# linjieli222/HERO

Measured on AMD Instinct MI355X. Metric: videos/sec training step, HERO-base TVR-shaped batch, higher is better.
Workload: dtype bf16; 1 GPU; configs[1]: HERO-base TVR finetune micro-step (train-tvr-8gpu.json shapes: 32 videos x 60 frames, 15 subs x (4 frames + 20 tokens), 15-token query; vfeat 4352; fwd + VSM loss + bwd, all-reduce/clip/AdamW every 2nd micro-step); global_batch=32, parallelism=dp1, grad_accum=2, launch=hipGraph replay, input=one batch resident in HBM

## Files before the change

hero_amd/_lib.py:

```python
import ctypes as C
import os

import torch

_HERE = os.path.dirname(os.path.abspath(__file__))
LIB_PATH = os.environ.get("HERO_HIP_LIB") or os.path.join(_HERE, "libhero_hip.so")

ABI_VERSION = 3
F32, BF16 = 0, 1
LAYOUT_K, LAYOUT_O = 0, 1
ACT_NONE, ACT_GELU, ACT_RELU, ACT_GELU_BWD, ACT_RELU_BWD, ACT_GELU_DG, ACT_MUL_AUX = 0, 1, 2, 3, 4, 5, 6

EXPORTS = [
    "hero_last_error", "hero_abi_version", "hero_abi_struct_count", "hero_abi_struct_bytes", "hero_gemm", "hero_gemm_splits", "hero_fold_slabs", "hero_wgrad_group", "hero_wgrad_batch_plan", "hero_wgrad_batch", "hero_prof_enable", "hero_prof_read", "hero_probe_mfma", "hero_probe_hbm", "hero_gemm_force_config", "hero_layernorm_fwd",
    "hero_layernorm_bwd_workspace_bytes", "hero_layernorm_bwd", "hero_colsum_workspace_bytes",
    "hero_colsum", "hero_colsum_multi", "hero_colsum_multi_workspace_bytes", "hero_layernorm_bwd_blocks", "hero_attention_fwd", "hero_attention_bwd", "hero_attention_max_len", "hero_attention_max_packed_len", "hero_attention_stats_ok", "hero_attention_force_ppw",
    "hero_gather_rows", "hero_inverse_first", "hero_csr_gather_sum", "hero_scatter_add_rows", "hero_segment_sort_workspace_bytes", "hero_scatter_add_sorted_workspace_bytes", "hero_segment_sort", "hero_scatter_add_sorted", "hero_cast", "hero_transpose_cast", "hero_copy_multi",
    "hero_relu_bwd", "hero_gelu_bwd", "hero_add", "hero_sumsq", "hero_adamw", "hero_adamw_multi", "hero_adamw_multi_chunk",
    "hero_query_pool_fwd", "hero_query_pool_bwd", "hero_rownorm_fwd", "hero_rownorm_bwd", "hero_score_max_fwd",
    "hero_score_max_bwd", "hero_rank_loss", "hero_sums_scaled", "hero_st_ed_fwd", "hero_st_ed_bwd", "hero_st_ed_bwd_workspace_bytes",
    "hero_cross_entropy_fwd", "hero_cross_entropy_bwd", "hero_qa_pool_fwd", "hero_qa_pool_bwd",
    "hero_topk_rows", "hero_st_ed_probs", "hero_moment_topk", "hero_moment_nms", "hero_first_hit",
    "hero_collate_subs", "hero_collate_clip_mask", "hero_collate_frame_map", "hero_collate_gather_feats", "hero_derive_multi",
    "hero_comm_available", "hero_comm_unique_id", "hero_comm_init", "hero_comm_destroy", "hero_comm_rank", "hero_comm_world",
    "hero_comm_allreduce_buckets", "hero_comm_broadcast", "hero_comm_allgather", "hero_comm_allgather_var",
]


class Dropout(C.Structure):
    _fields_ = [("seed_ptr", C.c_void_p), ("site", C.c_uint64),
                ("threshold16", C.c_uint32), ("scale", C.c_float)]


class GemmEpilogue(C.Structure):
    _fields_ = [("bias", C.c_void_p), ("residual", C.c_void_p), ("aux", C.c_void_p),
                ("act", C.c_int), ("out_f32", C.c_int), ("beta", C.c_float),
                ("split_k", C.c_int), ("dropout", Dropout), ("colsum", C.c_void_p), ("colsum_partial", C.c_int), ("pad_", C.c_int), ("split_stride", C.c_longlong)]


class CrossEntropy(C.Structure):
    _fields_ = [("logits", C.c_void_p), ("labels", C.c_void_p), ("loss", C.c_void_p), ("lse", C.c_void_p),
                ("dloss", C.c_void_p), ("dlogits", C.c_void_p), ("rows", C.c_int), ("cols", C.c_int),
                ("ld", C.c_int), ("dtype", C.c_int), ("inv_temp", C.c_float), ("ignore_index", C.c_int64)]


class Derive(C.Structure):
    _fields_ = [("src", C.c_void_p), ("dst", C.c_void_p), ("n", C.c_int64), ("mode", C.c_int), ("p0", C.c_int),
                ("p1", C.c_int), ("p2", C.c_int)]

# ... 113 lines not shown
    return {st.__name__: C.sizeof(st) for st in ABI_STRUCTS}


_lib = None


def lib():
    global _lib
    if _lib is None:
        if not os.path.exists(LIB_PATH):
            raise RuntimeError(
                "hero_amd: %s is missing. Build it with `python -m hero_amd.build` "
                "(needs hipcc; cross-compiles for gfx950 without a GPU). There is no fallback "
                "path." % LIB_PATH)
        L = C.CDLL(LIB_PATH)
        L.hero_last_error.restype = C.c_char_p
        have = L.hero_abi_version()
        if have != ABI_VERSION:
            raise RuntimeError("hero_amd: %s reports ABI version %d, this binding was written against %d (struct layouts "
                               "differ: rebuild with `python -m hero_amd.build --force`)" % (LIB_PATH, have, ABI_VERSION))
        L.hero_abi_struct_bytes.argtypes = [C.c_int]
        if L.hero_abi_struct_count() != len(ABI_STRUCTS):
            raise RuntimeError("hero_amd: %s declares %d ABI structs, this binding mirrors %d" % (LIB_PATH, L.hero_abi_struct_count(), len(ABI_STRUCTS)))
        bad = [(st.__name__, C.sizeof(st), L.hero_abi_struct_bytes(i)) for i, st in enumerate(ABI_STRUCTS)
               if C.sizeof(st) != L.hero_abi_struct_bytes(i)]
        if bad:
            raise RuntimeError("hero_amd: struct layouts differ from %s (name, binding bytes, library bytes): %s" % (LIB_PATH, bad))
        L.hero_layernorm_bwd_workspace_bytes.restype = C.c_size_t
        L.hero_colsum_workspace_bytes.restype = C.c_size_t
        L.hero_colsum_multi_workspace_bytes.restype = C.c_size_t
        L.hero_colsum_multi_workspace_bytes.argtypes = [C.POINTER(Colsum), C.c_int]
        L.hero_colsum_multi.argtypes = [C.POINTER(Colsum), C.c_int, C.c_void_p, C.c_void_p]
        L.hero_layernorm_bwd_blocks.argtypes = [C.c_int]
        L.hero_gemm.argtypes = [C.c_void_p, C.c_void_p, C.c_void_p] + [C.c_int] * 9 + [
            C.POINTER(GemmEpilogue), C.c_void_p]
        L.hero_gemm_splits.argtypes = [C.c_int, C.c_int, C.c_int]
        L.hero_fold_slabs.argtypes = [C.c_void_p, C.c_int, C.c_size_t, C.c_void_p, C.c_size_t, C.c_int, C.c_void_p]
        L.hero_wgrad_group.argtypes = [C.POINTER(WgradProblem), C.c_int, C.c_int, C.c_int, C.c_void_p]
        L.hero_wgrad_batch_plan.argtypes = [C.POINTER(WgradProblem), C.c_int, C.c_int, C.c_void_p, C.c_int]
        L.hero_wgrad_batch.argtypes = [C.POINTER(WgradProblem), C.c_int, C.c_int, C.c_int, C.c_void_p, C.c_int, C.c_void_p]
        L.hero_prof_enable.argtypes = [C.c_int]
        L.hero_prof_read.argtypes = [C.c_int, C.POINTER(C.c_double), C.POINTER(C.c_double),
                                     C.POINTER(C.c_longlong)]
        L.hero_probe_mfma.argtypes = [C.c_void_p, C.c_size_t, C.POINTER(C.c_double), C.POINTER(C.c_double), C.c_void_p]
        L.hero_probe_hbm.argtypes = [C.c_void_p, C.c_void_p, C.c_size_t, C.POINTER(C.c_double), C.POINTER(C.c_double), C.c_void_p]
        L.hero_layernorm_fwd.argtypes = [C.POINTER(LnFwd), C.c_void_p]
        L.hero_layernorm_bwd.argtypes = [C.POINTER(LnBwd), C.c_void_p]
        L.hero_layernorm_bwd_workspace_bytes.argtypes = [C.c_int, C.c_int]
        L.hero_colsum_workspace_bytes.argtypes = [C.c_int, C.c_int]
        L.hero_colsum.argtypes = [C.c_void_p, C.c_void_p, C.c_int, C.c_int, C.c_int, C.c_int,
                                  C.c_float, C.c_void_p, C.c_void_p]
        L.hero_attention_fwd.argtypes = [C.POINTER(Attn), C.c_void_p]
        L.hero_attention_bwd.argtypes = [C.POINTER(Attn), C.c_void_p]
        L.hero_attention_stats_ok.argtypes = [C.c_int, C.c_int]
        L.hero_attention_force_ppw.argtypes = [C.c_int]
        L.hero_attention_max_len.argtypes = [C.c_int, C.c_int]
        L.hero_attention_max_packed_len.argtypes = [C.c_int]
        L.hero_gather_rows.argtypes = [C.c_void_p, C.c_void_p, C.c_void_p, C.c_void_p,
                                       C.c_int, C.c_int, C.c_int, C.c_void_p]
        L.hero_inverse_first.argtypes = [C.c_void_p, C.c_int, C.c_void_p, C.c_int, C.c_int, C.c_void_p]
        L.hero_csr_gather_sum.argtypes = [C.c_void_p, C.c_void_p, C.c_void_p, C.c_void_p,
                                          C.c_int, C.c_int, C.c_int, C.c_void_p]
        L.hero_scatter_add_rows.argtypes = [C.c_void_p, C.c_void_p, C.c_void_p, C.c_void_p,
                                            C.c_int, C.c_int, C.c_int, C.c_int, C.c_int, C.c_void_p]
        L.hero_segment_sort_workspace_bytes.argtypes = [C.c_int]
        L.hero_segment_sort_workspace_bytes.restype = C.c_size_t
# ... 88 lines not shown
```

hero_amd/csrc/layernorm.hip:

```cpp
#include "common.h"

namespace hero {

__device__ __forceinline__ void add4(float4& s, const float4& v) { s.x += v.x; s.y += v.y; s.z += v.z; s.w += v.w; }
__device__ __forceinline__ void ln_mask4(float4& v, const DropCtx& drop, int row, int cols, int c) {
  const float4 m = drop.mask4(((uint64_t)row * (uint64_t)cols + (uint64_t)c) >> 2);
  v.x *= m.x; v.y *= m.y; v.z *= m.z; v.w *= m.w;
}

template <int VPL, int GRP>
__device__ __forceinline__ void ln_fwd_gamma_beta(const HeroLnFwd& a, const int (&cc)[VPL], int i0, float4 (&g)[GRP], float4 (&b)[GRP]) {
#pragma unroll
  for (int u = 0; u < GRP; ++u)
    if (i0 + u < VPL) {
      g[u] = *reinterpret_cast<const float4*>(a.gamma + cc[i0 + u]);
      b[u] = *reinterpret_cast<const float4*>(a.beta + cc[i0 + u]);
    }
}

template <typename TX, typename TY, int VPL, bool FULL>
__device__ __forceinline__ void ln_fwd_row(const HeroLnFwd& a, int row, int lane) {
  const int cols = FULL ? VPL * 256 : a.cols;
  int cc[VPL];
  float okf[VPL];
// ... 60 lines not shown
        const int i = i0 + u;
        o[u].x = (v[i].x - mean) * rstd * g[u].x + b[u].x;
        o[u].y = (v[i].y - mean) * rstd * g[u].y + b[u].y;
        o[u].z = (v[i].z - mean) * rstd * g[u].z + b[u].z;
        o[u].w = (v[i].w - mean) * rstd * g[u].w + b[u].w;
      }
    if (drop.on()) {
#pragma unroll
      for (int u = 0; u < GRP; ++u)
        if (i0 + u < VPL) ln_mask4(o[u], drop, row, cols, cc[i0 + u]);
    }
    if (pre) {
#pragma unroll
      for (int u = 0; u < GRP; ++u)
        if (i0 + u < VPL && (FULL || okf[i0 + u] != 0.f)) V4<TY>::st(pre + cc[i0 + u], v[i0 + u]);
    }
#pragma unroll
    for (int u = 0; u < GRP; ++u)
      if (i0 + u < VPL && (FULL || okf[i0 + u] != 0.f)) V4<TY>::st(y + cc[i0 + u], o[u]);
  }
}

template <typename TX, typename TY, int VPL>
__global__ __launch_bounds__(256) void ln_fwd_kernel(HeroLnFwd a) {
  const int lane = threadIdx.x & 63, row = blockIdx.x * 4 + (threadIdx.x >> 6);
  if (row < a.rows) ln_fwd_row<TX, TY, VPL, false>(a, row, lane);
}
template <typename TX, typename TY, int VPL>
__global__ __launch_bounds__(256) void ln_fwd_full_kernel(HeroLnFwd a) {
  const int lane = threadIdx.x & 63, row = blockIdx.x * 4 + (threadIdx.x >> 6);
  if (row < a.rows) ln_fwd_row<TX, TY, VPL, true>(a, row, lane);
}

template <typename TX, typename T, int VPL, bool FULL, bool ACC>
__device__ __forceinline__ void ln_bwd_row(const HeroLnBwd& a, int row, int lane, const DropCtx dout, const DropCtx din,
                                           const float4* gm, float4* ag, float4* ab, float4* ai) {
  const int cols = FULL ? VPL * 256 : a.cols;
  const float inv = 1.f / (float)cols;
  const TX* x = static_cast<const TX*>(a.x) + (size_t)row * cols;
  const T* dy = static_cast<const T*>(a.dy) + (size_t)row * cols;
  float4 xv[VPL], d[VPL];
  if constexpr (FULL) {
#pragma unroll
    for (int i = 0; i < VPL; ++i) {
      xv[i] = V4<TX>::ld(x + (lane + 64 * i) * 4);
      d[i] = V4<T>::ld(dy + (lane + 64 * i) * 4);
    }
  }
  const float mean = a.mean[row], rstd = a.rstd[row];
  if constexpr (FULL) {
    if (dout.on()) {
#pragma unroll
      for (int i = 0; i < VPL; ++i) ln_mask4(d[i], dout, row, cols, (lane + 64 * i) * 4);
    }
  }
  float4 xh[VPL], g[VPL];
  float s1 = 0.f, s2 = 0.f;
#pragma unroll
  for (int i = 0; i < VPL; ++i) {
    const int c = (lane + 64 * i) * 4;
    xh[i] = make_float4(0.f, 0.f, 0.f, 0.f);
    g[i] = xh[i];
    if (FULL || c < cols) {
      if constexpr (!FULL) {
        xv[i] = V4<TX>::ld(x + c);
        d[i] = V4<T>::ld(dy + c);
        if (dout.on()) ln_mask4(d[i], dout, row, cols, c);
      }
      const float4 gv = FULL ? gm[i] : *reinterpret_cast<const float4*>(a.gamma + c);
      xh[i] = make_float4((xv[i].x - mean) * rstd, (xv[i].y - mean) * rstd, (xv[i].z - mean) * rstd, (xv[i].w - mean) * rstd);
      g[i] = make_float4(d[i].x * gv.x, d[i].y * gv.y, d[i].z * gv.z, d[i].w * gv.w);
      if constexpr (ACC) {
        ag[i].x += d[i].x * xh[i].x; ag[i].y += d[i].y * xh[i].y; ag[i].z += d[i].z * xh[i].z; ag[i].w += d[i].w * xh[i].w;
        add4(ab[i], d[i]);
      }
      s1 += (g[i].x + g[i].y) + (g[i].z + g[i].w);
      s2 += (g[i].x * xh[i].x + g[i].y * xh[i].y) + (g[i].z * xh[i].z + g[i].w * xh[i].w);
    }
  }
  s1 = wave_sum(s1) * inv;
  s2 = wave_sum(s2) * inv;
  T* dx = a.dx ? static_cast<T*>(a.dx) + (size_t)row * cols : nullptr;
  T* dxd = a.dx_dropped ? static_cast<T*>(a.dx_dropped) + (size_t)row * cols : nullptr;
  constexpr int GRP = FULL ? VPL : 1;
#pragma unroll
  for (int i0 = 0; i0 < VPL; i0 += GRP) {
    if (!FULL && (lane + 64 * i0) * 4 >= cols) continue;
    float4 o[GRP];
#pragma unroll
    for (int u = 0; u < GRP; ++u) {
      const int i = i0 + u;
      o[u].x = rstd * (g[i].x - s1 - xh[i].x * s2);
      o[u].y = rstd * (g[i].y - s1 - xh[i].y * s2);
      o[u].z = rstd * (g[i].z - s1 - xh[i].z * s2);
      o[u].w = rstd * (g[i].w - s1 - xh[i].w * s2);
    }
    if (dx) {
#pragma unroll
      for (int u = 0; u < GRP; ++u) V4<T>::st(dx + (lane + 64 * (i0 + u)) * 4, o[u]);
    }
    if (din.on()) {
#pragma unroll
      for (int u = 0; u < GRP; ++u) ln_mask4(o[u], din, row, cols, (lane + 64 * (i0 + u)) * 4);
    }
    if (dxd) {
#pragma unroll
      for (int u = 0; u < GRP; ++u) V4<T>::st(dxd + (lane + 64 * (i0 + u)) * 4, o[u]);
    }
    if constexpr (ACC) {
#pragma unroll
      for (int u = 0; u < GRP; ++u) add4(ai[i0 + u], o[u]);
    }
  }
}

template <typename TX, typename T, int VPL>
__global__ __launch_bounds__(256) void ln_bwd_dx_kernel(HeroLnBwd a) {
  const int lane = threadIdx.x & 63, row = blockIdx.x * 4 + (threadIdx.x >> 6);
  if (row >= a.rows) return;
  DropCtx dout(a.dropout_out), din(a.dropout_in);
  ln_bwd_row<TX, T, VPL, false, false>(a, row, lane, dout, din, nullptr, nullptr, nullptr, nullptr);
}

template <typename TX, typename T, int VPL, bool FULL>
__device__ __forceinline__ void ln_bwd_fused(const HeroLnBwd& a, float* partial) {
  extern __shared__ __attribute__((aligned(16))) float red[];
  const int lane = threadIdx.x & 63, wave = threadIdx.x >> 6;
  const int cols = FULL ? VPL * 256 : a.cols;
  DropCtx dout(a.dropout_out), din(a.dropout_in);
  float4 ag[VPL], ab[VPL], ai[VPL], gm[VPL];
#pragma unroll
  for (int i = 0; i < VPL; ++i) {
    ag[i] = ab[i] = ai[i] = make_float4(0.f, 0.f, 0.f, 0.f);
    if constexpr (FULL) gm[i] = *reinterpret_cast<const float4*>(a.gamma + (lane + 64 * i) * 4);
  }
  for (int row = blockIdx.x * 4 + wave; row < a.rows; row += gridDim.x * 4)
    ln_bwd_row<TX, T, VPL, FULL, true>(a, row, lane, dout, din, gm, ag, ab, ai);
#pragma unroll
  for (int i = 0; i < VPL; ++i) {
    const int c = (lane + 64 * i) * 4;
    if (FULL || c < cols) {
      *reinterpret_cast<float4*>(red + ((size_t)(wave * 3 + 0)) * cols + c) = ag[i];
      *reinterpret_cast<float4*>(red + ((size_t)(wave * 3 + 1)) * cols + c) = ab[i];
      *reinterpret_cast<float4*>(red + ((size_t)(wave * 3 + 2)) * cols + c) = ai[i];
    }
  }
  __syncthreads();
  const int n4 = 3 * (cols >> 2);
  for (int q = threadIdx.x; q < n4; q += 256) {
    const int k = q / (cols >> 2), c = (q - k * (cols >> 2)) * 4;
    float4 v = *reinterpret_cast<const float4*>(red + (size_t)k * cols + c);
#pragma unroll
    for (int w = 1; w < 4; ++w) add4(v, *reinterpret_cast<const float4*>(red + ((size_t)(w * 3 + k)) * cols + c));
    *reinterpret_cast<float4*>(partial + ((size_t)blockIdx.x * 3 + k) * cols + c) = v;
  }
}

template <typename TX, typename T, int VPL>
__global__ __launch_bounds__(256) void ln_bwd_fused_kernel(HeroLnBwd a, float* partial) {
  ln_bwd_fused<TX, T, VPL, false>(a, partial);
}
template <typename TX, typename T, int VPL>
__global__ __launch_bounds__(256) __attribute__((amdgpu_waves_per_eu(4, 8))) void ln_bwd_fused_full_kernel(HeroLnBwd a, float* partial) {
  ln_bwd_fused<TX, T, VPL, true>(a, partial);
}

__global__ __launch_bounds__(256) void colred_final3_kernel(const float* partial, float* o0, float* o1, float* o2, int cols,
                                                            int nblocks, float beta) {
  const int k = blockIdx.y;
  float* out = k == 0 ? o0 : (k == 1 ? o1 : o2);
  if (!out) return;
  __shared__ float4 red[16][16];
  const int cg = threadIdx.x & 15, kl = threadIdx.x >> 4;
  const int c = (blockIdx.x * 16 + cg) * 4;
  float4 s = make_float4(0.f, 0.f, 0.f, 0.f);
  if (c < cols) {
    int b = kl;
    for (; b + 48 < nblocks; b += 64) {
      float4 v[4];
#pragma unroll
      for (int u = 0; u < 4; ++u) v[u] = *reinterpret_cast<const float4*>(partial + ((size_t)(b + 16 * u) * 3 + k) * cols + c);
#pragma unroll
      for (int u = 0; u < 4; ++u) add4(s, v[u]);
    }
    for (; b < nblocks; b += 16) add4(s, *reinterpret_cast<const float4*>(partial + ((size_t)b * 3 + k) * cols + c));
  }
  red[kl][cg] = s;
  __syncthreads();
  if (kl == 0 && c < cols) {
    float4 o = make_float4(0.f, 0.f, 0.f, 0.f);
    if (beta != 0.f) {
      o = *reinterpret_cast<const float4*>(out + c);
      o.x *= beta; o.y *= beta; o.z *= beta; o.w *= beta;
    }
#pragma unroll
    for (int j = 1; j < 16; ++j) add4(s, red[j][cg]);
    add4(o, s);
// ... 138 lines not shown
}

template <typename F>
static int ln_dtypes(const char* who, const char* second, int xd, int d, F f) {
  if (xd == HERO_F32 && d == HERO_F32) return f(float(), float());
  if (xd == HERO_F32 && d == HERO_BF16) return f(float(), bf16_t());
  if (xd == HERO_BF16 && d == HERO_BF16) return f(bf16_t(), bf16_t());
  set_error("%s: unsupported dtypes x=%d %s=%d", who, xd, second, d);
  return HERO_ERR_UNSUPPORTED;
}

#define HERO_VPL_SWITCH4(cols, CALL)                                       \
  do {                                                                     \
    const int need4 = ((cols) + 255) / 256;                                \
    if (need4 <= 1) { CALL(1); }                                           \
    else if (need4 <= 2) { CALL(2); }                                      \
    else if (need4 <= 3) { CALL(3); }                                      \
    else { CALL(4); }                                                      \
  } while (0)
#define HERO_VPL_SWITCH(cols, CALL)                                        \
  do {                                                                     \
    const int need = ((cols) + 255) / 256;                                 \
    if (need <= 4) HERO_VPL_SWITCH4(cols, CALL);                           \
    else if (need <= 6) { CALL(6); }                                       \
    else if (need <= 8) { CALL(8); }                                       \
    else if (need <= 12) { CALL(12); }                                     \
    else if (need <= 17) { CALL(17); }                                     \
    else if (need <= 24) { CALL(24); }                                     \
    else { set_error("layernorm: cols %d too wide (max 6144)", (cols)); return HERO_ERR_UNSUPPORTED; } \
  } while (0)

}

#define LN_BWD_MAX_BLOCKS 1024
using namespace hero;

extern "C" int hero_layernorm_fwd(const HeroLnFwd* a, hero_stream_t stream) {
  HERO_REQUIRE(a && a->y && a->gamma && a->beta, "hero_layernorm_fwd: null pointer");
  HERO_REQUIRE(a->x || a->tab[0] || a->tab[1] || a->tab[2], "hero_layernorm_fwd: no input");
  HERO_REQUIRE(a->cols > 0 && a->cols % 4 == 0, "hero_layernorm_fwd: cols (%d) must be a positive multiple of 4", a->cols);
  if (a->rows <= 0) return HERO_OK;
  hipStream_t s = static_cast<hipStream_t>(stream);
  const dim3 grid((a->rows + 3) / 4), block(256);
  const int xd = a->x ? a->x_dtype : a->y_dtype, yd = a->y_dtype;
  int rc = HERO_OK;
#define LAUNCH(KERNEL, V)                                                                         \
  rc = ln_dtypes("hero_layernorm_fwd", "y", xd, yd, [&](auto tx, auto ty) {                       \
    hipLaunchKernelGGL((KERNEL<decltype(tx), decltype(ty), V>), grid, block, 0, s, *a);           \
    return HERO_OK;                                                                               \
  })
  if (a->x && !a->tab[0] && !a->tab[1] && !a->tab[2] && a->cols % 256 == 0 && a->cols <= 1024) {
#define CALL(V) LAUNCH(ln_fwd_full_kernel, V)
    HERO_VPL_SWITCH4(a->cols, CALL);
#undef CALL
    return rc ? rc : check_launch("hero_layernorm_fwd(full)");
  }
#define CALL(V) LAUNCH(ln_fwd_kernel, V)
  HERO_VPL_SWITCH(a->cols, CALL);
#undef CALL
#undef LAUNCH
  return rc ? rc : check_launch("hero_layernorm_fwd");
}

extern "C" size_t hero_layernorm_bwd_workspace_bytes(int rows, int cols) {
  (void)rows;
  return (size_t)LN_BWD_MAX_BLOCKS * (size_t)cols * 3 * sizeof(float);
}
extern "C" size_t hero_colsum_workspace_bytes(int rows, int cols) {
  (void)rows;
  return (size_t)256 * (size_t)cols * sizeof(float);
}

extern "C" int hero_layernorm_bwd(const HeroLnBwd* a, hero_stream_t stream) {
  HERO_REQUIRE(a && a->x && a->dy && a->gamma && a->mean && a->rstd, "hero_layernorm_bwd: null pointer");
  HERO_REQUIRE(a->cols > 0 && a->cols % 4 == 0, "hero_layernorm_bwd: cols (%d) must be a positive multiple of 4", a->cols);
  if (a->rows <= 0) return HERO_OK;
  hipStream_t s = static_cast<hipStream_t>(stream);
  const int xd = a->x_dtype, d = a->dtype;
  const bool want_params = a->dgamma || a->dbeta || a->dbias_in;
  if (want_params) HERO_REQUIRE(a->workspace, "hero_layernorm_bwd: workspace required for parameter gradients");
  int rc = HERO_OK;
#define LAUNCH(KERNEL, V, LDS, ...)                                                                         \
  rc = ln_dtypes("hero_layernorm_bwd", "dy", xd, d, [&](auto tx, auto t) {                                  \
    hipLaunchKernelGGL((KERNEL<decltype(tx), decltype(t), V>), grid, block, LDS, s, __VA_ARGS__);          \
    return HERO_OK;                                                                                         \
  })
  if (want_params && (a->dx || a->dx_dropped || a->dbias_in) && a->cols <= 1024) {
    int nblk = (a->rows + 3) / 4;
    if (nblk > LN_BWD_MAX_BLOCKS) nblk = LN_BWD_MAX_BLOCKS;
    float* partial = static_cast<float*>(a->workspace);
    const size_t lds = (size_t)4 * 3 * a->cols * sizeof(float);
    const dim3 grid(nblk), block(256);
    if (a->cols % 256 == 0) {
#define CALL(V) LAUNCH(ln_bwd_fused_full_kernel, V, lds, *a, partial)
      HERO_VPL_SWITCH4(a->cols, CALL);
#undef CALL
    } else {
#define CALL(V) LAUNCH(ln_bwd_fused_kernel, V, lds, *a, partial)
      HERO_VPL_SWITCH4(a->cols, CALL);
#undef CALL
    }
    if (rc) return rc;
    rc = check_launch("hero_layernorm_bwd(fused)");
    if (rc || a->defer_fold) return rc;
    hipLaunchKernelGGL(colred_final3_kernel, dim3((a->cols + 63) / 64, 3), dim3(256), 0, s, partial, a->dgamma, a->dbeta,
                       a->dbias_in, a->cols, nblk, a->grad_beta);
    return check_launch("hero_layernorm_bwd(final3)");
  }
  HERO_REQUIRE(!a->dbias_in, "hero_layernorm_bwd: dbias_in needs cols <= 1024");
  HERO_REQUIRE(!a->defer_fold, "hero_layernorm_bwd: defer_fold needs the fused path (cols <= 1024, dx or dbias_in wanted)");
  if (a->dx || a->dx_dropped) {
    const dim3 grid((a->rows + 3) / 4), block(256);
#define CALL(V) LAUNCH(ln_bwd_dx_kernel, V, 0, *a)
    HERO_VPL_SWITCH(a->cols, CALL);
#undef CALL
    if (rc) return rc;
    rc = check_launch("hero_layernorm_bwd(dx)");
    if (rc) return rc;
  }
#undef LAUNCH
  if (a->dgamma || a->dbeta)
    return ln_dtypes("hero_layernorm_bwd", "dy", xd, d, [&](auto tx, auto t) {
      return run_colred<decltype(tx), decltype(t)>(a->x, a->dy, a->mean, a->rstd, a->dgamma, a->dbeta, a->rows, a->cols, a->cols,
                                                   a->grad_beta, a->dropout_out, a->workspace, s);
    });
  return HERO_OK;
}

extern "C" int hero_layernorm_bwd_blocks(int rows) {
  int nblk = (rows + 3) / 4;
  return nblk > LN_BWD_MAX_BLOCKS ? LN_BWD_MAX_BLOCKS : nblk;
}

struct ColsumMulti {
  HeroColsum p[HERO_COLSUM_MULTI_MAX];
  int blk0[HERO_COLSUM_MULTI_MAX + 1];
  int woff[HERO_COLSUM_MULTI_MAX];
  int rpc[HERO_COLSUM_MULTI_MAX];
  int n;
};

__device__ __forceinline__ int colsum_find(const ColsumMulti& a, int b) {
  int lo = 0, hi = a.n - 1;
  while (lo < hi) {
    const int mid = (lo + hi + 1) >> 1;
    if (a.blk0[mid] <= b) lo = mid; else hi = mid - 1;
  }
  return lo;
}

__global__ __launch_bounds__(256) void colsum_multi_part_kernel(ColsumMulti a, float* ws) {
  __shared__ float4 red[4][64];
  const int pi = colsum_find(a, blockIdx.x);
  const HeroColsum P = a.p[pi];
  const int ncb = (P.cols + 255) / 256;
  const int local = blockIdx.x - a.blk0[pi], cb = local % ncb, chunk = local / ncb;
  const int tx = threadIdx.x & 63, ty = threadIdx.x >> 6;
  const int c = (cb * 64 + tx) * 4;
  const int r0 = chunk * a.rpc[pi], r1 = min(P.rows, r0 + a.rpc[pi]);
  float4 s = make_float4(0.f, 0.f, 0.f, 0.f), unused = s;
  const float* const none = nullptr;
  if (c < P.cols) {
    if (P.dtype == HERO_BF16) colsum_chunk(static_cast<const bf16_t*>(P.src), P.ld, c, r0, r1, ty, s, none, none, none, 0, nullptr, unused);
    else colsum_chunk(static_cast<const float*>(P.src), P.ld, c, r0, r1, ty, s, none, none, none, 0, nullptr, unused);
// ... 98 lines not shown
```

hero_amd/functional.py:

```python
import ctypes as C
import math
import os
import weakref

import numpy as np
import torch

from . import _lib as L

_COMPUTE_DTYPE = torch.bfloat16


def set_compute_dtype(dtype):
    global _COMPUTE_DTYPE
    if dtype not in (torch.float32, torch.bfloat16):
        raise ValueError("compute dtype must be torch.float32 or torch.bfloat16")
    _COMPUTE_DTYPE = dtype


def compute_dtype():
    return _COMPUTE_DTYPE


class _Rng:
# ... 274 lines not shown
        k_gemm(L.ptr(dy2) + 2 * n1, L.ptr(Wt) + 2 * n1, L.ptr(slabs) + 4 * n_main * stride, M, K, N - n1, N, N, K,
               L.LAYOUT_K, L.LAYOUT_K, L.BF16, out_f32=True)
    out = torch.empty((M, K), dtype=torch.bfloat16, device=dy2.device)
    L.check(L.lib().hero_fold_slabs(L.ptr(slabs), slabs.shape[0], stride, L.ptr(out), stride, L.BF16, L.stream()))
    return out


def _split_for(n_out, n_in, rows, bk):
    tiles = ((n_out + 127) // 128) * ((n_in + 127) // 128)
    ktiles = max(1, -(-rows // bk))
    flops = 2.0 * n_out * n_in * rows
    out_bytes = 4.0 * n_out * n_in
    best, best_t = 1, None
    for s in range(1, 17):
        if s > 1 and ktiles // s < 4:
            break
        blocks = tiles * s
        rounds = -(-blocks // 512)
        last = blocks - (rounds - 1) * 512
        t = flops / blocks * ((rounds - 1) / 1.83e12 + (1 / 2.7e12 if last <= 256 else 1 / 1.83e12))
        if s > 1:
            t += out_bytes * s / 2.0e12
        if best_t is None or t < best_t:
            best, best_t = s, t
    return best


_WQ = []
_WQ_TASK = [-1]
GROUP_WGRADS = [True]
WGRAD_BATCH = [32]
WGRAD_DBIAS_RIDE = [True]
WGRAD_RIDE_MAX_ROWS = [1 << 30]
B1_EPILOGUE = [False]
B1_PARTIALS = [True]
WGRAD_QUEUE_BYTES = [int(os.environ.get("HERO_WGRAD_QUEUE_MB", "4096")) << 20]
_WQ_BYTES = [0]
_WPLANS = {}
_WPLANS_PINNED = set()


def _wgrad_queue_full(device):
    if _WQ_BYTES[0] <= WGRAD_QUEUE_BYTES[0]:
        return False
    hard = _WQ_HARD.get(device.index)
    if hard is None:
        env = os.environ.get("HERO_WGRAD_QUEUE_HARD_MB")
        hard = (int(env) << 20) if env else max(2 * WGRAD_QUEUE_BYTES[0], int(0.15 * torch.cuda.get_device_properties(device).total_memory))
        _WQ_HARD[device.index] = hard
    if _WQ_BYTES[0] > hard:
        return True
    tiles = sum(-(-e[4] // 192) * -(-e[1].shape[1] // 192) for e in _WQ)
    full, rem = divmod(tiles, 256)
    if rem == 0:
        return True
    p = -(-rem // 8)
    slices = max(1, min(32 // p, 8))
    return tiles / 256.0 >= 0.9 * (full + (1.4 if slices > 1 else 1.0) / slices)


_WQ_HARD = {}


def _wgrad_limit():
    return 4 if (WGRAD_BATCH[0] <= 4 or SINK.wants_overlap()) else min(WGRAD_BATCH[0], 32)

# ... 184 lines not shown
    if weight is not None and weight.requires_grad:
        k_wgrad(dy2, x2, out=SINK.dst(weight), beta=1.0, col0=col0, ncols=N, on_done=lambda: SINK.done(weight),
                dbias=SINK.dst(bias) if want_b else None, dbias_done=(lambda: SINK.done(bias)) if want_b else None)
    elif want_b:
        k_colsum(dy2, out=SINK.dst(bias), beta=1.0, col0=col0, ncols=N, on_done=lambda: SINK.done(bias))


def k_ln_fwd(x2, gamma, beta, eps, out_dtype, rows, cols, tabs=(), idxs=(), want_pre=False,
             drop=None, device=None):
    device = device or (x2.device if x2 is not None else gamma.device)
    y = torch.empty((rows, cols), dtype=out_dtype, device=device)
    mean = torch.empty((rows,), dtype=torch.float32, device=device)
    rstd = torch.empty((rows,), dtype=torch.float32, device=device)
    pre = torch.empty((rows, cols), dtype=out_dtype, device=device) if want_pre else None
    a = L.LnFwd()
    a.x = L.ptr(x2)
    for k in range(3):
        a.tab[k] = L.ptr(tabs[k]) if k < len(tabs) else None
        a.idx[k] = L.ptr(idxs[k]) if k < len(idxs) and idxs[k] is not None else None
    a.gamma, a.beta, a.y, a.pre = L.ptr(gamma), L.ptr(beta), L.ptr(y), L.ptr(pre)
    a.mean, a.rstd = L.ptr(mean), L.ptr(rstd)
    a.rows, a.cols, a.eps = rows, cols, eps
    a.x_dtype = L.dt(x2) if x2 is not None else L.dt(y)
    a.y_dtype = L.dt(y)
    a.dropout = _d(drop)
    L.check(L.lib().hero_layernorm_fwd(C.byref(a), L.stream()))
    return y, mean, rstd, pre


def ln_param_dsts(gamma_p, beta_p):
    dg = SINK.dst(gamma_p) if gamma_p.requires_grad else None
    db = SINK.dst(beta_p) if beta_p.requires_grad else None
    return dg, db


def ln_params_done(gamma_p, beta_p):
    if gamma_p.requires_grad:
        SINK.done(gamma_p)
    if beta_p.requires_grad:
        SINK.done(beta_p)


def k_ln_bwd(x2, dy2, gamma, mean, rstd, want_dx=True, want_params=True, drop_out=None,
             drop_in=None, dgamma=None, dbeta=None, grad_beta=0.0, dbias_in=None):
    rows, cols = dy2.shape
    dev = dy2.device
    dx = torch.empty_like(dy2) if want_dx else None
    dxd = torch.empty_like(dy2) if (want_dx and drop_in is not None) else None
    dg, db = dgamma, dbeta
    if want_params and dg is None and db is None:
        dg = torch.empty((cols,), dtype=torch.float32, device=dev)
        db = torch.empty((cols,), dtype=torch.float32, device=dev)
    ws = _workspace(3072 * cols, dev) if (dg is not None or db is not None or dbias_in is not None) else None
    defer = (grad_beta == 1.0 and ws is not None and cols <= 1024 and (want_dx or dbias_in is not None) and _colsum_defer_ok())
    if defer:
        nblk = L.lib().hero_layernorm_bwd_blocks(rows)
        ws = torch.empty((nblk, 3 * cols), dtype=torch.float32, device=dev)
    a = L.LnBwd()
    a.x, a.dy, a.gamma, a.mean, a.rstd = L.ptr(x2), L.ptr(dy2), L.ptr(gamma), L.ptr(mean), L.ptr(rstd)
    a.dx, a.dx_dropped, a.dgamma, a.dbeta = L.ptr(dx), L.ptr(dxd), L.ptr(dg), L.ptr(db)
    a.grad_beta, a.workspace = grad_beta, L.ptr(ws)
    a.rows, a.cols, a.x_dtype, a.dtype = rows, cols, L.dt(x2), L.dt(dy2)
    a.dropout_out, a.dropout_in = _d(drop_out), _d(drop_in)
    a.dbias_in = L.ptr(dbias_in)
    a.defer_fold = 1 if defer else 0
    L.check(L.lib().hero_layernorm_bwd(C.byref(a), L.stream()))
# ... 638 lines not shown
        ctx.save_for_backward(x2, packed_t((wq, wk, wv), x2.dtype), qkv, probs, ctxt)
        return ctxt.view(S, Lq, D)

    @staticmethod
    def backward(ctx, dctx):
        x2, Wqkv_t, qkv, probs, ctxt = ctx.saved_tensors
        S, Lq, H, D = ctx.dims
        dqkv = k_attn_bwd(qkv, probs, _as2d(dctx), S, Lq, H, drop=ctx.drop, ctx=ctxt, mask_add=ctx.mask_add)
        dx = k_dgrad_t(dqkv, Wqkv_t).view(S, Lq, D) if ctx.needs_input_grad[0] else None
        _qkv_bwd(dqkv, x2, ctx.params, D)
        return (dx,) + (None,) * 9


class ProjResLnFn(torch.autograd.Function):

    @staticmethod
    def forward(ctx, h, res, eps, drop, w, b, gamma, beta):
        h2, r2 = _as2d(h), _as2d(res)
        Wc = packed((w,), h2.dtype)
        y = k_linear(h2, Wc, b.detach(), residual=r2, drop=drop)
        out, mean, rstd, _ = k_ln_fwd(y, gamma.detach(), beta.detach(), eps, y.dtype, y.shape[0], y.shape[1])
        ctx.drop = drop
        ctx.hshape, ctx.rshape = h.shape, res.shape
        ctx.params = (w, b, gamma, beta)
        _use(*ctx.params)
        ctx.save_for_backward(h2, packed_t((w,), h2.dtype), y, mean, rstd, gamma.detach())
        return out.view(res.shape)

    @staticmethod
    def backward(ctx, dout):
        h2, Wt, y, mean, rstd, gamma = ctx.saved_tensors
        w, b, gp, bp = ctx.params
        dgd, dbd = ln_param_dsts(gp, bp)
        fuse_b = b.requires_grad and y.shape[1] <= 1024
        dy, dyd, _, _ = k_ln_bwd(y, _as2d(dout), gamma, mean, rstd, drop_in=ctx.drop, dgamma=dgd,
                                 dbeta=dbd, grad_beta=1.0, want_params=False,
                                 dbias_in=SINK.dst(b) if fuse_b else None)
        ln_params_done(gp, bp)
        if fuse_b:
            SINK.done(b)
        acc_linear_grads(dyd, h2, w, None if fuse_b else b)
        dh = k_dgrad_t(dyd, Wt).view(ctx.hshape)
        return (dh, dy.view(ctx.rshape)) + (None,) * 6


ONE_ATTN_LAUNCH = [True]
_SEQ_OFF = {}


def _one_attention_launch(segs, masks, drops, x2):
    if not (ONE_ATTN_LAUNCH[0] and len(segs) > 1 and all(len(sg) == 2 for sg in segs) and x2.dtype == torch.bfloat16 and x2.is_cuda):
        return segs, masks, drops
    lmax = max(sg[1] for sg in segs)
    if ATTN_SAVE_PROBS or not L.lib().hero_attention_stats_ok(L.BF16, lmax) or any(m is not None and m.requires_grad for m in masks):
        return segs, masks, drops
    key = (tuple(segs), x2.device.index)
    off = _SEQ_OFF.get(key)
    if off is None:
        o, r = [0], 0
        for S_, L_ in segs:
            for _ in range(S_):
                r += L_
                o.append(r)
        off = _SEQ_OFF[key] = torch.tensor(o, dtype=torch.int32, device=x2.device)
    if all(m is None for m in masks):
        mcat = None
    else:
# ... 18 lines not shown
        Wo = packed((wo,), x2.dtype)
        qkv = k_linear(x2, Wqkv, bqkv)
        ctxt = torch.empty((x2.shape[0], D), dtype=x2.dtype, device=x2.device)
        segs, masks, drops_attn = _one_attention_launch(segs, masks, drops_attn, x2)
        probs = []
        r0 = 0
        for seg, m, dr in zip(segs, masks, drops_attn):
            if len(seg) == 4:
                _, S, Lq, off = seg
                _, p = k_attn_fwd(qkv, m, S, Lq, H, drop=dr, out=ctxt, seq_off=off)
                probs.append(p)
                continue
            S, Lq = seg
            _, p = k_attn_fwd(qkv[r0:r0 + S * Lq], m, S, Lq, H, drop=dr, out=ctxt[r0:r0 + S * Lq])
            probs.append(p)
            r0 += S * Lq
        y1 = k_linear(ctxt, Wo, bo.detach(), residual=x2, drop=drop_hid)
        a, mean, rstd, _ = k_ln_fwd(y1, g1.detach(), b1.detach(), eps, y1.dtype, x2.shape[0], D)
        ctx.meta = (segs, H, D, drops_attn, drop_hid, x.shape)
        ctx.masks = masks
        ctx.params = (wq, bq, wk, bk, wv, bv, wo, bo, g1, b1)
        _use(*ctx.params)
        ctx.save_for_backward(x2, packed_t((wq, wk, wv), x2.dtype), packed_t((wo,), x2.dtype), qkv, ctxt, y1,
                              mean, rstd, g1.detach(), *probs)
        return a.view(x.shape)

    @staticmethod
    def backward(ctx, da):
        x2, Wqkv_t, Wo_t, qkv, ctxt, y1, mean, rstd, g1 = ctx.saved_tensors[:9]
        probs = ctx.saved_tensors[9:]
        segs, H, D, drops_attn, drop_hid, xshape = ctx.meta
        wq, bq, wk, bk, wv, bv, wo, bo, g1p, b1p = ctx.params
        dgd, dbd = ln_param_dsts(g1p, b1p)
        fuse_b = bo.requires_grad and D <= 1024
        dy1, dy1d, _, _ = k_ln_bwd(y1, _as2d(da), g1, mean, rstd, drop_in=drop_hid, dgamma=dgd,
                                   dbeta=dbd, grad_beta=1.0, want_params=False,
                                   dbias_in=SINK.dst(bo) if fuse_b else None)
        ln_params_done(g1p, b1p)
        if fuse_b:
            SINK.done(bo)
        acc_linear_grads(dy1d, ctxt, wo, None if fuse_b else bo)
        dctx = k_dgrad_t(dy1d, Wo_t)
        dqkv = torch.empty_like(qkv)
        r0 = 0
        for seg, p, dr, m in zip(segs, probs, drops_attn, ctx.masks):
            if len(seg) == 4:
                _, S, Lq, off = seg
                k_attn_bwd(qkv, p, dctx, S, Lq, H, drop=dr, out=dqkv, seq_off=off, ctx=ctxt, mask_add=m)
                continue
            S, Lq = seg
            k_attn_bwd(qkv[r0:r0 + S * Lq], p, dctx[r0:r0 + S * Lq], S, Lq, H, drop=dr,
                       out=dqkv[r0:r0 + S * Lq], ctx=ctxt[r0:r0 + S * Lq], mask_add=m)
            r0 += S * Lq
        _qkv_bwd(dqkv, x2, (wq, bq, wk, bk, wv, bv), D)
        dx = k_dgrad_t(dqkv, Wqkv_t, residual=dy1).view(xshape)
        return (dx,) + (None,) * 16


class FfnBlockFn(torch.autograd.Function):

    @staticmethod
    def forward(ctx, a, eps, drop_hid, w1, b1, w2, b2, g2, bt2):
        shp = a.shape
        a2 = _as2d(a)
        W1, W2 = packed((w1,), a2.dtype), packed((w2,), a2.dtype)
        u = torch.empty((a2.shape[0], W1.shape[0]), dtype=a2.dtype, device=a2.device)
        hg = k_linear(a2, W1, b1.detach(), act=L.ACT_GELU_DG, aux=u)
        y2 = k_linear(hg, W2, b2.detach(), residual=a2, drop=drop_hid)
        out, mean, rstd, _ = k_ln_fwd(y2, g2.detach(), bt2.detach(), eps, y2.dtype, y2.shape[0], y2.shape[1])
        ctx.drop, ctx.shp = drop_hid, shp
        ctx.params = (w1, b1, w2, b2, g2, bt2)
        _use(*ctx.params)
        ctx.save_for_backward(a2, packed_t((w1,), a2.dtype), packed_t((w2,), a2.dtype), u, hg, y2, mean,
                              rstd, g2.detach())
        return out.view(shp)

    @staticmethod
    def backward(ctx, dout):
        a2, W1_t, W2_t, u, hg, y2, mean, rstd, g2 = ctx.saved_tensors
        w1, b1, w2, b2, g2p, bt2p = ctx.params
        dgd, dbd = ln_param_dsts(g2p, bt2p)
        fuse_b = b2.requires_grad and y2.shape[1] <= 1024
        dy2, dy2d, _, _ = k_ln_bwd(y2, _as2d(dout), g2, mean, rstd, drop_in=ctx.drop, dgamma=dgd,
                                   dbeta=dbd, grad_beta=1.0, want_params=False,
                                   dbias_in=SINK.dst(b2) if fuse_b else None)
        ln_params_done(g2p, bt2p)
        if fuse_b:
            SINK.done(b2)
        acc_linear_grads(dy2d, hg, w2, None if fuse_b else b2)
        part = None
        if b1.requires_grad and B1_PARTIALS[0] and dy2d.dtype == torch.bfloat16:
            part = torch.empty((-(-dy2d.shape[0] // 64), W2_t.shape[0]), dtype=torch.float32, device=dy2d.device)
        fuse_b1 = part is None and b1.requires_grad and (SINK.wants_overlap() or not GROUP_WGRADS[0] or B1_EPILOGUE[0])
        du = k_dgrad_t(dy2d, W2_t, act=L.ACT_MUL_AUX, aux=u,
                       colsum=part if part is not None else (SINK.dst(b1) if fuse_b1 else None), colsum_partial=part is not None)
        if part is not None:
            k_colsum(part, out=SINK.dst(b1), beta=1.0, on_done=lambda: SINK.done(b1))
        acc_linear_grads(du, a2, w1, None if (fuse_b1 or part is not None) else b1)
        if fuse_b1:
            SINK.done(b1)
        da = k_dgrad_t(du, W1_t, residual=dy2).view(ctx.shp)
        return (da,) + (None,) * 8
```

include/hero_hip.h:

```cpp
#ifndef HERO_HIP_H_
#define HERO_HIP_H_

#include <stddef.h>
#include <stdint.h>

#ifdef __cplusplus
extern "C" {
#endif

typedef void* hero_stream_t;

enum { HERO_F32 = 0, HERO_BF16 = 1 };
enum { HERO_OK = 0, HERO_ERR_ARG = -1, HERO_ERR_LAUNCH = -2, HERO_ERR_UNSUPPORTED = -3 };

const char* hero_last_error(void);
#define HERO_ABI_VERSION 3
int hero_abi_version(void);
enum { HERO_STRUCT_DROPOUT = 0, HERO_STRUCT_GEMM_EPILOGUE, HERO_STRUCT_WGRAD_PROBLEM, HERO_STRUCT_LN_FWD, HERO_STRUCT_LN_BWD,
       HERO_STRUCT_COLSUM, HERO_STRUCT_ATTN, HERO_STRUCT_ADAMW, HERO_STRUCT_TENSOR_DESC, HERO_STRUCT_ADAMW_GROUP,
       HERO_STRUCT_ADAMW_MULTI, HERO_STRUCT_COPY_DESC, HERO_STRUCT_QUERY_POOL, HERO_STRUCT_ROW_NORM, HERO_STRUCT_SCORE_MAX,
       HERO_STRUCT_RANK_LOSS, HERO_STRUCT_ST_ED, HERO_STRUCT_CROSS_ENTROPY, HERO_STRUCT_DERIVE, HERO_STRUCT_COMM_BUCKET,
       HERO_STRUCT_COUNT_ };
int hero_abi_struct_count(void);
int hero_abi_struct_bytes(int which);
// ... 63 lines not shown
  const float* beta;
  void* y;
  void* pre;
  float* mean;
  float* rstd;
  int rows, cols;
  float eps;
  int x_dtype, y_dtype;
  HeroDropout dropout;
} HeroLnFwd;
int hero_layernorm_fwd(const HeroLnFwd* a, hero_stream_t stream);

typedef struct HeroLnBwd {
  const void* x;
  const void* dy;
  const float* gamma;
  const float* mean;
  const float* rstd;
  void* dx;
  void* dx_dropped;
  float* dgamma;
  float* dbeta;
  float grad_beta;
  void* workspace;
  int rows, cols;
  int x_dtype, dtype;
  HeroDropout dropout_out;
  HeroDropout dropout_in;
  float* dbias_in;
  int defer_fold;
} HeroLnBwd;
size_t hero_layernorm_bwd_workspace_bytes(int rows, int cols);
int hero_layernorm_bwd_blocks(int rows);
int hero_layernorm_bwd(const HeroLnBwd* a, hero_stream_t stream);

size_t hero_colsum_workspace_bytes(int rows, int cols);
int hero_colsum(const void* x, float* out, int rows, int cols, int ld, int dtype, float beta,
                void* workspace, hero_stream_t stream);
#define HERO_COLSUM_MULTI_MAX 64
typedef struct HeroColsum {
  const void* src;
  float* dst;
  int rows, cols, ld, dtype;
  float beta;
  int row_cols;
  const int32_t* dst_rows;
} HeroColsum;
size_t hero_colsum_multi_workspace_bytes(const HeroColsum* p, int n);
int hero_colsum_multi(const HeroColsum* p, int n, void* workspace, hero_stream_t stream);

typedef struct HeroAttn {
  const void* qkv;
  const float* mask;
  void* ctx;
  float* probs;
  const void* dctx;
  void* dqkv;
  int S, L, H;
  float scale;
  int dtype;
  HeroDropout dropout;
  const int32_t* seq_off;
  float* stats;
} HeroAttn;
int hero_attention_fwd(const HeroAttn* a, hero_stream_t stream);
int hero_attention_bwd(const HeroAttn* a, hero_stream_t stream);
// ... 240 lines not shown
```

Before: 5228 videos/s.

## Pipeline row loads in fused LayerNorm backward and widen its blocks

```diff
diff --git a/hero_amd/_lib.py b/hero_amd/_lib.py
--- a/hero_amd/_lib.py
+++ b/hero_amd/_lib.py
@@ -14,7 +14,7 @@
 EXPORTS = [
     "hero_last_error", "hero_abi_version", "hero_abi_struct_count", "hero_abi_struct_bytes", "hero_gemm", "hero_gemm_splits", "hero_fold_slabs", "hero_wgrad_group", "hero_wgrad_batch_plan", "hero_wgrad_batch", "hero_prof_enable", "hero_prof_read", "hero_probe_mfma", "hero_probe_hbm", "hero_gemm_force_config", "hero_layernorm_fwd",
     "hero_layernorm_bwd_workspace_bytes", "hero_layernorm_bwd", "hero_colsum_workspace_bytes",
-    "hero_colsum", "hero_colsum_multi", "hero_colsum_multi_workspace_bytes", "hero_layernorm_bwd_blocks", "hero_attention_fwd", "hero_attention_bwd", "hero_attention_max_len", "hero_attention_max_packed_len", "hero_attention_stats_ok", "hero_attention_force_ppw",
+    "hero_colsum", "hero_colsum_multi", "hero_colsum_multi_workspace_bytes", "hero_layernorm_bwd_blocks", "hero_layernorm_bwd_waves", "hero_attention_fwd", "hero_attention_bwd", "hero_attention_max_len", "hero_attention_max_packed_len", "hero_attention_stats_ok", "hero_attention_force_ppw",
     "hero_gather_rows", "hero_inverse_first", "hero_csr_gather_sum", "hero_scatter_add_rows", "hero_segment_sort_workspace_bytes", "hero_scatter_add_sorted_workspace_bytes", "hero_segment_sort", "hero_scatter_add_sorted", "hero_cast", "hero_transpose_cast", "hero_copy_multi",
     "hero_relu_bwd", "hero_gelu_bwd", "hero_add", "hero_sumsq", "hero_adamw", "hero_adamw_multi", "hero_adamw_multi_chunk",
     "hero_query_pool_fwd", "hero_query_pool_bwd", "hero_rownorm_fwd", "hero_rownorm_bwd", "hero_score_max_fwd",
@@ -194,6 +194,7 @@
         L.hero_colsum_multi_workspace_bytes.argtypes = [C.POINTER(Colsum), C.c_int]
         L.hero_colsum_multi.argtypes = [C.POINTER(Colsum), C.c_int, C.c_void_p, C.c_void_p]
         L.hero_layernorm_bwd_blocks.argtypes = [C.c_int]
+        L.hero_layernorm_bwd_waves.argtypes = [C.c_int, C.c_int]
         L.hero_gemm.argtypes = [C.c_void_p, C.c_void_p, C.c_void_p] + [C.c_int] * 9 + [
             C.POINTER(GemmEpilogue), C.c_void_p]
         L.hero_gemm_splits.argtypes = [C.c_int, C.c_int, C.c_int]
diff --git a/hero_amd/csrc/layernorm.hip b/hero_amd/csrc/layernorm.hip
--- a/hero_amd/csrc/layernorm.hip
+++ b/hero_amd/csrc/layernorm.hip
@@ -116,27 +116,65 @@
   if (row < a.rows) ln_fwd_row<TX, TY, VPL, true>(a, row, lane);
 }
 
-template <typename TX, typename T, int VPL, bool FULL, bool ACC>
+template <typename T> struct Raw4;
+template <> struct Raw4<float> {
+  typedef float4 type;
+  static __device__ __forceinline__ type ld(const float* p) { return *reinterpret_cast<const float4*>(p); }
+  static __device__ __forceinline__ float4 cvt(type r) { return r; }
+};
+template <> struct Raw4<bf16_t> {
+  typedef uint2 type;
+  static __device__ __forceinline__ type ld(const bf16_t* p) { return *reinterpret_cast<const uint2*>(p); }
+  static __device__ __forceinline__ float4 cvt(type u) {
+    return make_float4(__uint_as_float(u.x << 16), __uint_as_float(u.x & 0xffff0000u), __uint_as_float(u.y << 16),
+                       __uint_as_float(u.y & 0xffff0000u));
+  }
+};
+
+template <typename TX, typename T, int VPL>
+struct LnBwdRaw {
+  typename Raw4<TX>::type x[VPL];
+  typename Raw4<T>::type d[VPL];
+  float mean, rstd;
+};
+template <typename TX, typename T, int VPL>
+__device__ __forceinline__ void ln_bwd_load(const HeroLnBwd& a, int row, int lane, LnBwdRaw<TX, T, VPL>& r) {
+  const TX* x = static_cast<const TX*>(a.x) + (size_t)row * (VPL * 256);
+  const T* dy = static_cast<const T*>(a.dy) + (size_t)row * (VPL * 256);
+#pragma unroll
+  for (int i = 0; i < VPL; ++i) {
+    r.x[i] = Raw4<TX>::ld(x + (lane + 64 * i) * 4);
+    r.d[i] = Raw4<T>::ld(dy + (lane + 64 * i) * 4);
+  }
+  r.mean = a.mean[row];
+  r.rstd = a.rstd[row];
+}
+
+template <typename TX, typename T, int VPL, bool FULL, bool ACC, bool DBIAS>
 __device__ __forceinline__ void ln_bwd_row(const HeroLnBwd& a, int row, int lane, const DropCtx dout, const DropCtx din,
-                                           const float4* gm, float4* ag, float4* ab, float4* ai) {
+                                           const float4* gm, float4* ag, float4* ab, float4* ai,
+                                           const LnBwdRaw<TX, T, VPL>* raw) {
   const int cols = FULL ? VPL * 256 : a.cols;
   const float inv = 1.f / (float)cols;
   const TX* x = static_cast<const TX*>(a.x) + (size_t)row * cols;
   const T* dy = static_cast<const T*>(a.dy) + (size_t)row * cols;
   float4 xv[VPL], d[VPL];
+  float mean, rstd;
   if constexpr (FULL) {
 #pragma unroll
     for (int i = 0; i < VPL; ++i) {
-      xv[i] = V4<TX>::ld(x + (lane + 64 * i) * 4);
-      d[i] = V4<T>::ld(dy + (lane + 64 * i) * 4);
-    }
-  }
-  const float mean = a.mean[row], rstd = a.rstd[row];
-  if constexpr (FULL) {
+      xv[i] = Raw4<TX>::cvt(raw->x[i]);
+      d[i] = Raw4<T>::cvt(raw->d[i]);
+    }
+    mean = raw->mean;
+    rstd = raw->rstd;
     if (dout.on()) {
 #pragma unroll
       for (int i = 0; i < VPL; ++i) ln_mask4(d[i], dout, row, cols, (lane + 64 * i) * 4);
     }
+  } else {
+    mean = a.mean[row];
+    rstd = a.rstd[row];
   }
   float4 xh[VPL], g[VPL];
   float s1 = 0.f, s2 = 0.f;
@@ -191,7 +229,7 @@
 #pragma unroll
       for (int u = 0; u < GRP; ++u) V4<T>::st(dxd + (lane + 64 * (i0 + u)) * 4, o[u]);
     }
-    if constexpr (ACC) {
+    if constexpr (ACC && DBIAS) {
 #pragma unroll
       for (int u = 0; u < GRP; ++u) add4(ai[i0 + u], o[u]);
     }
@@ -203,50 +241,82 @@
   const int lane = threadIdx.x & 63, row = blockIdx.x * 4 + (threadIdx.x >> 6);
   if (row >= a.rows) return;
   DropCtx dout(a.dropout_out), din(a.dropout_in);
-  ln_bwd_row<TX, T, VPL, false, false>(a, row, lane, dout, din, nullptr, nullptr, nullptr, nullptr);
-}
-
-template <typename TX, typename T, int VPL, bool FULL>
+  ln_bwd_row<TX, T, VPL, false, false, false>(a, row, lane, dout, din, nullptr, nullptr, nullptr, nullptr, nullptr);
+}
+
+template <typename TX, typename T, int VPL, bool FULL, int W, bool DBIAS>
 __device__ __forceinline__ void ln_bwd_fused(const HeroLnBwd& a, float* partial) {
+  constexpr int NS = DBIAS ? 3 : 2;
   extern __shared__ __attribute__((aligned(16))) float red[];
   const int lane = threadIdx.x & 63, wave = threadIdx.x >> 6;
   const int cols = FULL ? VPL * 256 : a.cols;
   DropCtx dout(a.dropout_out), din(a.dropout_in);
-  float4 ag[VPL], ab[VPL], ai[VPL], gm[VPL];
+  float4 ag[VPL], ab[VPL], ai[DBIAS ? VPL : 1], gm[VPL];
 #pragma unroll
   for (int i = 0; i < VPL; ++i) {
-    ag[i] = ab[i] = ai[i] = make_float4(0.f, 0.f, 0.f, 0.f);
+    ag[i] = ab[i] = make_float4(0.f, 0.f, 0.f, 0.f);
+    if constexpr (DBIAS) ai[i] = ag[i];
     if constexpr (FULL) gm[i] = *reinterpret_cast<const float4*>(a.gamma + (lane + 64 * i) * 4);
   }
-  for (int row = blockIdx.x * 4 + wave; row < a.rows; row += gridDim.x * 4)
-    ln_bwd_row<TX, T, VPL, FULL, true>(a, row, lane, dout, din, gm, ag, ab, ai);
+  const int stride = gridDim.x * W;
+  int row = blockIdx.x * W + wave;
+  if constexpr (FULL) {
+#ifdef LN_BWD_NO_PIPE
+    constexpr bool PIPE = false;
+#else
+    constexpr bool PIPE = VPL < 4;
+#endif
+    LnBwdRaw<TX, T, VPL> cur;
+    if (PIPE && row < a.rows) ln_bwd_load(a, row, lane, cur);
+#pragma unroll
+    for (int i = 0; i < VPL; ++i) asm volatile("" ::"v"(gm[i].x), "v"(gm[i].y), "v"(gm[i].z), "v"(gm[i].w));
+    while (row < a.rows) {
+      const int next = row + stride;
+      if constexpr (PIPE) {
+        LnBwdRaw<TX, T, VPL> nxt = cur;
+        if (next < a.rows) ln_bwd_load(a, next, lane, nxt);
+        ln_bwd_row<TX, T, VPL, true, true, DBIAS>(a, row, lane, dout, din, gm, ag, ab, ai, &cur);
+        cur = nxt;
+      } else {
+        ln_bwd_load(a, row, lane, cur);
+        ln_bwd_row<TX, T, VPL, true, true, DBIAS>(a, row, lane, dout, din, gm, ag, ab, ai, &cur);
+      }
+      row = next;
+    }
+  } else {
+    for (; row < a.rows; row += stride)
+      ln_bwd_row<TX, T, VPL, false, true, DBIAS>(a, row, lane, dout, din, gm, ag, ab, ai, nullptr);
+  }
 #pragma unroll
   for (int i = 0; i < VPL; ++i) {
     const int c = (lane + 64 * i) * 4;
     if (FULL || c < cols) {
-      *reinterpret_cast<float4*>(red + ((size_t)(wave * 3 + 0)) * cols + c) = ag[i];
-      *reinterpret_cast<float4*>(red + ((size_t)(wave * 3 + 1)) * cols + c) = ab[i];
-      *reinterpret_cast<float4*>(red + ((size_t)(wave * 3 + 2)) * cols + c) = ai[i];
+      *reinterpret_cast<float4*>(red + ((size_t)(wave * NS + 0)) * cols + c) = ag[i];
+      *reinterpret_cast<float4*>(red + ((size_t)(wave * NS + 1)) * cols + c) = ab[i];
+      if constexpr (DBIAS) *reinterpret_cast<float4*>(red + ((size_t)(wave * NS + 2)) * cols + c) = ai[i];
     }
   }
   __syncthreads();
-  const int n4 = 3 * (cols >> 2);
-  for (int q = threadIdx.x; q < n4; q += 256) {
+  const int n4 = NS * (cols >> 2);
+  for (int q = threadIdx.x; q < n4; q += 64 * W) {
     const int k = q / (cols >> 2), c = (q - k * (cols >> 2)) * 4;
     float4 v = *reinterpret_cast<const float4*>(red + (size_t)k * cols + c);
 #pragma unroll
-    for (int w = 1; w < 4; ++w) add4(v, *reinterpret_cast<const float4*>(red + ((size_t)(w * 3 + k)) * cols + c));
+    for (int w = 1; w < W; ++w) add4(v, *reinterpret_cast<const float4*>(red + ((size_t)(w * NS + k)) * cols + c));
     *reinterpret_cast<float4*>(partial + ((size_t)blockIdx.x * 3 + k) * cols + c) = v;
   }
 }
 
-template <typename TX, typename T, int VPL>
-__global__ __launch_bounds__(256) void ln_bwd_fused_kernel(HeroLnBwd a, float* partial) {
-  ln_bwd_fused<TX, T, VPL, false>(a, partial);
-}
-template <typename TX, typename T, int VPL>
-__global__ __launch_bounds__(256) __attribute__((amdgpu_waves_per_eu(4, 8))) void ln_bwd_fused_full_kernel(HeroLnBwd a, float* partial) {
-  ln_bwd_fused<TX, T, VPL, true>(a, partial);
+#ifndef LN_BWD_OCC
+#define LN_BWD_OCC 3
+#endif
+template <typename TX, typename T, int VPL, int W, bool DBIAS>
+__global__ __launch_bounds__(64 * W) __attribute__((amdgpu_waves_per_eu(LN_BWD_OCC, 8))) void ln_bwd_fused_kernel(HeroLnBwd a, float* partial) {
+  ln_bwd_fused<TX, T, VPL, false, W, DBIAS>(a, partial);
+}
+template <typename TX, typename T, int VPL, int W, bool DBIAS>
+__global__ __launch_bounds__(64 * W) __attribute__((amdgpu_waves_per_eu(LN_BWD_OCC, 8))) void ln_bwd_fused_full_kernel(HeroLnBwd a, float* partial) {
+  ln_bwd_fused<TX, T, VPL, true, W, DBIAS>(a, partial);
 }
 
 __global__ __launch_bounds__(256) void colred_final3_kernel(const float* partial, float* o0, float* o1, float* o2, int cols,
@@ -451,7 +521,19 @@
 
 }
 
+#ifndef LN_BWD_W
+#define LN_BWD_W (LN_BWD_OCC * 4)
+#endif
+#ifndef LN_BWD_CAP
+#define LN_BWD_CAP (256 * (LN_BWD_OCC * 4 / LN_BWD_W))
+#endif
 #define LN_BWD_MAX_BLOCKS 1024
+static inline int ln_bwd_blocks(int rows) {
+  const int nblk = (rows + LN_BWD_W - 1) / LN_BWD_W;
+  return nblk > LN_BWD_CAP ? LN_BWD_CAP : nblk;
+}
+static_assert(LN_BWD_CAP <= LN_BWD_MAX_BLOCKS, "the partials must fit the workspace");
+static_assert((size_t)LN_BWD_W * 3 * 1024 * sizeof(float) <= 160 * 1024, "LDS of the widest row");
 using namespace hero;
 
 extern "C" int hero_layernorm_fwd(const HeroLnFwd* a, hero_stream_t stream) {
@@ -505,20 +587,33 @@
     return HERO_OK;                                                                                         \
   })
   if (want_params && (a->dx || a->dx_dropped || a->dbias_in) && a->cols <= 1024) {
-    int nblk = (a->rows + 3) / 4;
-    if (nblk > LN_BWD_MAX_BLOCKS) nblk = LN_BWD_MAX_BLOCKS;
+    constexpr int W = LN_BWD_W;
+    const int nblk = ln_bwd_blocks(a->rows);
     float* partial = static_cast<float*>(a->workspace);
-    const size_t lds = (size_t)4 * 3 * a->cols * sizeof(float);
-    const dim3 grid(nblk), block(256);
+    const size_t lds = (size_t)W * (a->dbias_in ? 3 : 2) * a->cols * sizeof(float);
+    const dim3 grid(nblk), block(64 * W);
+#define FUSED(KERNEL, V, DB)                                                                                \
+  rc = ln_dtypes("hero_layernorm_bwd", "dy", xd, d, [&](auto tx, auto t) -> int {                           \
+    auto* kern = &KERNEL<decltype(tx), decltype(t), V, W, DB>;                                              \
+    if (lds > 65536) HERO_ENSURE_LDS(kern, W * 3 * V * 256 * sizeof(float), #KERNEL);                       \
+    hipLaunchKernelGGL(kern, grid, block, lds, s, *a, partial);                                             \
+    return HERO_OK;                                                                                         \
+  })
+#define FUSED_W(KERNEL, V)                                                                                  \
+  do {                                                                                                      \
+    if (a->dbias_in) FUSED(KERNEL, V, true); else FUSED(KERNEL, V, false);                                  \
+  } while (0)
     if (a->cols % 256 == 0) {
-#define CALL(V) LAUNCH(ln_bwd_fused_full_kernel, V, lds, *a, partial)
+#define CALL(V) FUSED_W(ln_bwd_fused_full_kernel, V)
       HERO_VPL_SWITCH4(a->cols, CALL);
 #undef CALL
     } else {
-#define CALL(V) LAUNCH(ln_bwd_fused_kernel, V, lds, *a, partial)
+#define CALL(V) FUSED_W(ln_bwd_fused_kernel, V)
       HERO_VPL_SWITCH4(a->cols, CALL);
 #undef CALL
     }
+#undef FUSED_W
+#undef FUSED
     if (rc) return rc;
     rc = check_launch("hero_layernorm_bwd(fused)");
     if (rc || a->defer_fold) return rc;
@@ -546,9 +641,11 @@
   return HERO_OK;
 }
 
-extern "C" int hero_layernorm_bwd_blocks(int rows) {
-  int nblk = (rows + 3) / 4;
-  return nblk > LN_BWD_MAX_BLOCKS ? LN_BWD_MAX_BLOCKS : nblk;
+extern "C" int hero_layernorm_bwd_blocks(int rows) { return ln_bwd_blocks(rows); }
+extern "C" int hero_layernorm_bwd_waves(int rows, int cols) {
+  (void)rows;
+  (void)cols;
+  return LN_BWD_W;
 }
 
 struct ColsumMulti {
diff --git a/hero_amd/functional.py b/hero_amd/functional.py
--- a/hero_amd/functional.py
+++ b/hero_amd/functional.py
@@ -330,6 +330,7 @@
 WGRAD_BATCH = [32]
 WGRAD_DBIAS_RIDE = [True]
 WGRAD_RIDE_MAX_ROWS = [1 << 30]
+LN_BIAS_RIDE = [True]
 B1_EPILOGUE = [False]
 B1_PARTIALS = [True]
 WGRAD_QUEUE_BYTES = [int(os.environ.get("HERO_WGRAD_QUEUE_MB", "4096")) << 20]
@@ -580,6 +581,14 @@
     dg = SINK.dst(gamma_p) if gamma_p.requires_grad else None
     db = SINK.dst(beta_p) if beta_p.requires_grad else None
     return dg, db
+
+
+def ln_fuses_bias(bias, weight, dy2):
+    if not (bias.requires_grad and dy2.shape[1] <= 1024):
+        return False
+    rides = (LN_BIAS_RIDE[0] and WGRAD_DBIAS_RIDE[0] and GROUP_WGRADS[0] and not SINK.wants_overlap() and weight.requires_grad
+             and dy2.dtype == torch.bfloat16 and dy2.shape[0] <= WGRAD_RIDE_MAX_ROWS[0] and torch._C._current_graph_task_id() != -1)
+    return not rides
 
 
 def ln_params_done(gamma_p, beta_p):
@@ -1284,7 +1293,7 @@
         h2, Wt, y, mean, rstd, gamma = ctx.saved_tensors
         w, b, gp, bp = ctx.params
         dgd, dbd = ln_param_dsts(gp, bp)
-        fuse_b = b.requires_grad and y.shape[1] <= 1024
+        fuse_b = ln_fuses_bias(b, w, y)
         dy, dyd, _, _ = k_ln_bwd(y, _as2d(dout), gamma, mean, rstd, drop_in=ctx.drop, dgamma=dgd,
                                  dbeta=dbd, grad_beta=1.0, want_params=False,
                                  dbias_in=SINK.dst(b) if fuse_b else None)
@@ -1369,7 +1378,7 @@
         segs, H, D, drops_attn, drop_hid, xshape = ctx.meta
         wq, bq, wk, bk, wv, bv, wo, bo, g1p, b1p = ctx.params
         dgd, dbd = ln_param_dsts(g1p, b1p)
-        fuse_b = bo.requires_grad and D <= 1024
+        fuse_b = ln_fuses_bias(bo, wo, y1)
         dy1, dy1d, _, _ = k_ln_bwd(y1, _as2d(da), g1, mean, rstd, drop_in=drop_hid, dgamma=dgd,
                                    dbeta=dbd, grad_beta=1.0, want_params=False,
                                    dbias_in=SINK.dst(bo) if fuse_b else None)
@@ -1417,7 +1426,7 @@
         a2, W1_t, W2_t, u, hg, y2, mean, rstd, g2 = ctx.saved_tensors
         w1, b1, w2, b2, g2p, bt2p = ctx.params
         dgd, dbd = ln_param_dsts(g2p, bt2p)
-        fuse_b = b2.requires_grad and y2.shape[1] <= 1024
+        fuse_b = ln_fuses_bias(b2, w2, y2)
         dy2, dy2d, _, _ = k_ln_bwd(y2, _as2d(dout), g2, mean, rstd, drop_in=ctx.drop, dgamma=dgd,
                                    dbeta=dbd, grad_beta=1.0, want_params=False,
                                    dbias_in=SINK.dst(b2) if fuse_b else None)
diff --git a/include/hero_hip.h b/include/hero_hip.h
--- a/include/hero_hip.h
+++ b/include/hero_hip.h
@@ -119,6 +119,7 @@
 } HeroLnBwd;
 size_t hero_layernorm_bwd_workspace_bytes(int rows, int cols);
 int hero_layernorm_bwd_blocks(int rows);
+int hero_layernorm_bwd_waves(int rows, int cols);
 int hero_layernorm_bwd(const HeroLnBwd* a, hero_stream_t stream);
 
 size_t hero_colsum_workspace_bytes(int rows, int cols);
```

Measured after the change: 5278 videos/s (median of 6 runs). No clear change (+1.0%).
